# facebookresearch/habitat-lab

Hardware: NVIDIA H100
Metric: DD-PPO learner frames/sec (ResNet18 RGB-D 256x256) (higher is better)
Workload: dtype bf16

## Files before the change

### habitat-lab_b200/csrc/conv.cu

```cuda
#include "common.cuh"
#include "wgmma.cuh"

namespace hb200 {
void count_launch(int n);
static int g_umma_layout = 1;

using namespace wg;

constexpr int kStages = 3;
constexpr int kTileM = 128;
constexpr int kMaxBN = 128;
constexpr int kChunkK = 64;
constexpr int kMaxChunks = 512;

template <int LAYOUT>
__device__ __forceinline__ uint32_t tile_off(int row, int k8, int rows_total) {
  if (LAYOUT == 0) return (uint32_t)(k8 * rows_total + row) << 4;
  return (uint32_t)((row >> 3) << 10) + (uint32_t)((row & 7) << 7) + (uint32_t)((k8 ^ (row & 7)) << 4);
}
template <int LAYOUT>
__device__ __forceinline__ uint64_t kmajor_desc(uint32_t base, int kk, int rows_total) {
  if (LAYOUT == 0)
    return make_smem_desc(base + (uint32_t)(kk * 2 * rows_total * 16), (uint32_t)rows_total * 16, 128, kNoSwizzle);
  return make_smem_desc(base + (uint32_t)(kk * 32), 16, 1024, kSwizzle128B);
}
template <int LAYOUT>
constexpr uint32_t kmajor_hi() { return LAYOUT == 0 ? 8 * 128 : 8 * 1024; }

struct ConvArgs {
  const __nv_bfloat16* src;
  const __nv_bfloat16* wimg;
  __nv_bfloat16* out;
  const __nv_bfloat16* addend;
  double* stats;
  int B, SH, SW, SC;
  int OH, OW, OC;
  int kh, kw, stride, pad;
  int M, nchunks, cshift, gn_groups;
  const float* bias;
  int relu;
  int s2_classes;
  int wbn;
};

template <int BN, int MODE, int LAYOUT, int NST = kStages>
__global__ void __launch_bounds__(128) conv_igemm_kernel(const ConvArgs a) {
  extern __shared__ __align__(16) uint8_t smem_raw[];
  constexpr uint32_t kABytes = kTileM * kChunkK * 2;
  constexpr uint32_t kBBytes = BN * kChunkK * 2;
  constexpr uint32_t kStageBytes = kABytes + kBBytes;
  static_assert(BN <= kMaxBN, "conv: N tile");
  static_assert(NST * kStageBytes >= kStageFloats * sizeof(float), "conv: epilogue transpose buffer");
  const uint32_t smem_base = (smem_u32(smem_raw) + 1023u) & ~1023u;
  float* const stage_buf = reinterpret_cast<float*>(smem_raw + (smem_base - smem_u32(smem_raw)));

  const int tid = threadIdx.x, lane = tid & 31;
  const int n0 = blockIdx.y * BN;
  __shared__ short chunk_ids[kMaxChunks];
  __shared__ int n_valid_s;
  int m, ob, op, oq, ph = 0, pw = 0;
  bool row_ok;
  if (MODE == 1 && a.s2_classes) {
    const int mq = a.M >> 2;
    const int tiles_per_class = (mq + kTileM - 1) / kTileM;
    const int cls = blockIdx.x / tiles_per_class;
    const int idx = (blockIdx.x - cls * tiles_per_class) * kTileM + tid;
    ph = cls >> 1; pw = cls & 1;
    row_ok = idx < mq;
    const int h2 = a.OH >> 1, w2 = a.OW >> 1;
    const int ii = row_ok ? idx : 0;
    ob = ii / (h2 * w2);
    const int rem = ii - ob * (h2 * w2);
    op = 2 * (rem / w2) + ph;
    oq = 2 * (rem % w2) + pw;
    m = (ob * a.OH + op) * a.OW + oq;
  } else {
    m = blockIdx.x * kTileM + tid;
    row_ok = m < a.M;
    const int hw = a.OH * a.OW;
    const int mm = row_ok ? m : 0;
    ob = mm / hw;
    const int rem = mm - ob * hw;
// ... 90 lines not shown
      if (MODE == 0) {
        ih = op * a.stride - a.pad + r;
        iw = oq * a.stride - a.pad + s;
        ok = ok && ih >= 0 && ih < a.SH && iw >= 0 && iw < a.SW;
      } else {
        const int th = op + a.pad - r, tw = oq + a.pad - s;
        ih = th / a.stride;
        iw = tw / a.stride;
        ok = ok && th >= 0 && tw >= 0 && (ih * a.stride == th) && (iw * a.stride == tw) &&
             ih < a.SH && iw < a.SW;
      }
      const __nv_bfloat16* g =
          ok ? a.src + ((((size_t)ob * a.SH + ih) * a.SW + iw) << a.cshift) + c0 : a.src;
      cp_async16(sa + tile_off<LAYOUT>(tid, j, kTileM), g, ok);
    }
    }
    const uint4* wsrc = reinterpret_cast<const uint4*>(wtile + (size_t)chunk * ((size_t)wbn * kChunkK));
#pragma unroll
    for (int i = 0; i < BN / 16; ++i) {
      const int v = tid + i * 128;
      cp_async16(sb + ((uint32_t)v << 4), wsrc + v, true);
    }
  };

  constexpr int kT = MODE == 0 ? kF16 : kBF16;
  float acc_t[BN];
#pragma unroll
  for (int c = 0; c < NST - 1; ++c) {
    if (c < n_valid) load_chunk(chunk_ids[c], c);
    cp_async_commit();
  }
  for (int c = 0; c < n_valid; ++c) {
    const int stage = c % NST;
    cp_async_wait<NST - 2>();
    fence_proxy_async_smem();
    __syncthreads();
    {
      const uint32_t sa = smem_base + stage * kStageBytes;
      const uint32_t sb = sa + kABytes;
      wgmma_fence();
#pragma unroll
      for (int kk = 0; kk < kChunkK / 16; ++kk)
        mma128<BN, kT>(acc_t, kmajor_desc<LAYOUT>(sa, kk, kTileM), kmajor_hi<LAYOUT>(), kmajor_desc<LAYOUT>(sb, kk, BN),
                       (c > 0 || kk > 0) ? 1u : 0u);
      wgmma_commit();
    }
    const int nc = c + NST - 1;
    if (nc < n_valid) {
      wgmma_wait<1>();
      load_chunk(chunk_ids[nc], nc % NST);
    }
    cp_async_commit();
  }
  wgmma_wait<0>();
  acc_fence(acc_t);

  const int hw = a.OH * a.OW;
  int seg = 1;
  if ((hw & (hw - 1)) == 0) seg = hw < 32 ? hw : 32;
#pragma unroll
  for (int col0 = 0; col0 < BN; col0 += 32) {
    float acc[32];
    if (n_valid > 0) {
      acc_row32(acc_t, col0, stage_buf, acc);
    } else {
#pragma unroll
      for (int j = 0; j < 32; ++j) acc[j] = 0.f;
    }

    if (MODE == 0 && a.stats != nullptr) {
      const int cpg = a.OC / a.gn_groups;
      float s2[16], q2[16];
#pragma unroll
      for (int i = 0; i < 16; ++i) {
        s2[i] = acc[2 * i] + acc[2 * i + 1];
        q2[i] = acc[2 * i] * acc[2 * i] + acc[2 * i + 1] * acc[2 * i + 1];
      }
      int lg = 0;
      while ((2 << lg) < cpg && lg < 4) ++lg;
#pragma unroll
      for (int lvl = 0; lvl < 4; ++lvl) {
        if (lvl < lg) {
#pragma unroll
          for (int i = 0; i < (8 >> lvl); ++i) {
            s2[i] = s2[2 * i] + s2[2 * i + 1];
            q2[i] = q2[2 * i] + q2[2 * i + 1];
          }
        }
      }
      const int ng = 16 >> lg;
#pragma unroll
      for (int off = 1; off < 32; off <<= 1) {
        if (off < seg) {
#pragma unroll
          for (int i = 0; i < 16; ++i) {
            if (i < ng) {
              s2[i] += __shfl_xor_sync(0xffffffffu, s2[i], off);
              q2[i] += __shfl_xor_sync(0xffffffffu, q2[i], off);
            }
          }
        }
      }
      if (row_ok && (lane & (seg - 1)) == 0) {
        const int g0 = (n0 + col0) / cpg;
        double* dst = a.stats + ((size_t)ob * a.gn_groups + g0) * 2;
#pragma unroll
        for (int i = 0; i < 16; ++i) {
          if (i < ng) {
            atomicAdd(dst + 2 * i, (double)s2[i]);
            atomicAdd(dst + 2 * i + 1, (double)q2[i]);
          }
        }
      }
    }
    if (MODE == 0 && a.bias != nullptr) {
#pragma unroll
      for (int j = 0; j < 32; ++j) acc[j] += __ldg(a.bias + n0 + col0 + j);
    }
    if (MODE == 0 && a.relu) {
#pragma unroll
      for (int j = 0; j < 32; ++j) acc[j] = fmaxf(acc[j], 0.f);
    }
    if (row_ok) {
      const size_t o = (size_t)m * a.OC + n0 + col0;
      if (MODE == 1 && a.addend != nullptr) {
        const uint4* ad = reinterpret_cast<const uint4*>(a.addend + o);
#pragma unroll
        for (int v = 0; v < 4; ++v) {
          float f[8];
          unpack8(ad[v], f);
#pragma unroll
          for (int e = 0; e < 8; ++e) acc[v * 8 + e] += f[e];
        }
      }
      uint4* dst = reinterpret_cast<uint4*>(a.out + o);
#pragma unroll
      for (int v = 0; v < 4; ++v) {
        uint4 u;
        if (MODE == 0) {
          u.x = pack_f16x2(acc[v * 8 + 0], acc[v * 8 + 1]);
          u.y = pack_f16x2(acc[v * 8 + 2], acc[v * 8 + 3]);
          u.z = pack_f16x2(acc[v * 8 + 4], acc[v * 8 + 5]);
          u.w = pack_f16x2(acc[v * 8 + 6], acc[v * 8 + 7]);
        } else {
          u.x = pack_bf16x2(acc[v * 8 + 0], acc[v * 8 + 1]);
          u.y = pack_bf16x2(acc[v * 8 + 2], acc[v * 8 + 3]);
          u.z = pack_bf16x2(acc[v * 8 + 4], acc[v * 8 + 5]);
          u.w = pack_bf16x2(acc[v * 8 + 6], acc[v * 8 + 7]);
        }
        dst[v] = u;
      }
    }
  }
}

struct WgradArgs {
  const __nv_bfloat16* x;
  const __nv_bfloat16* dy;
  float* dw;
  int B, Hi, Wi, Ci, Ho, Wo, Co, kh, kw, stride, pad;
  int P;
  int KW;
  int chunks_per_split;
  int cshift;
};

template <int BN>
__global__ void __launch_bounds__(128) conv_wgrad_kernel(const WgradArgs a) {
  extern __shared__ __align__(16) uint8_t smem_raw[];
  __shared__ float stage_buf[kStageFloats];
  constexpr uint32_t kABytes = kTileM * kChunkK * 2;
  constexpr uint32_t kBBytes = BN * kChunkK * 2;
  constexpr uint32_t kStageBytes = kABytes + kBBytes;
  constexpr uint32_t kLboA = (kTileM / 8) * 128, kLboB = (BN / 8) * 128;
  static_assert(BN <= kMaxBN, "conv_wgrad: N tile");
  const uint32_t smem_base = (smem_u32(smem_raw) + 1023u) & ~1023u;

  const int tid = threadIdx.x;
  const int row_base = blockIdx.x * kTileM;
  const int n0 = blockIdx.y * BN;
  const long long total_chunks = ((long long)a.P + kChunkK - 1) / kChunkK;
  const long long c_begin = (long long)blockIdx.z * a.chunks_per_split;
  long long c_end = c_begin + a.chunks_per_split;
  if (c_end > total_chunks) c_end = total_chunks;
  const int nchunks = (int)(c_end - c_begin);
  if (nchunks <= 0) return;

  const int kpix = tid & 63;
  const int half = tid >> 6;
  const int taps = a.kh * a.kw;
  const int hw = a.Ho * a.Wo;

  auto load_chunk = [&](int chunk, int stage) {
    const uint32_t sa = smem_base + stage * kStageBytes;
    const uint32_t sb = sa + kABytes;
    const long long pg = (c_begin + chunk) * kChunkK + kpix;
    const bool pix_ok = pg < a.P;
    int b = 0, oh = 0, ow = 0;
    if (pix_ok) {
      b = (int)(pg / hw);
      const int rem = (int)(pg - (long long)b * hw);
      oh = rem / a.Wo;
      ow = rem - oh * a.Wo;
    }
    const uint32_t koff = (uint32_t)(kpix >> 3) * 0 + (uint32_t)((kpix & 7) << 4);
#pragma unroll
    for (int i = 0; i < 8; ++i) {
      const int mb = half * 8 + i;
      const int row0 = row_base + mb * 8;
      const int tap = row0 >> a.cshift;
      const int c0 = row0 & (a.Ci - 1);
      const int r = tap / a.kw, s = tap - r * a.kw;
      const int ih = oh * a.stride - a.pad + r, iw = ow * a.stride - a.pad + s;
      const bool ok = pix_ok && tap < taps && ih >= 0 && ih < a.Hi && iw >= 0 && iw < a.Wi;
      const __nv_bfloat16* g = ok ? a.x + ((((size_t)b * a.Hi + ih) * a.Wi + iw) << a.cshift) + c0 : a.x;
      cp_async16(sa + (uint32_t)(kpix >> 3) * kLboA + (uint32_t)mb * 128 + koff, g, ok);
    }
#pragma unroll
    for (int i = 0; i < BN / 16; ++i) {
      const int nb = half + 2 * i;
      const __nv_bfloat16* g = pix_ok ? a.dy + (size_t)pg * a.Co + n0 + nb * 8 : a.dy;
      cp_async16(sb + (uint32_t)(kpix >> 3) * kLboB + (uint32_t)nb * 128 + koff, g, pix_ok);
    }
  };

  float acc_t[BN];
#pragma unroll
  for (int c = 0; c < kStages - 1; ++c) {
    if (c < nchunks) load_chunk(c, c);
    cp_async_commit();
  }
  for (int c = 0; c < nchunks; ++c) {
    const int stage = c % kStages;
    cp_async_wait<kStages - 2>();
// ... 104 lines not shown
    for (int col0 = 0; col0 < N; col0 += 32) {
      float r[32];
      acc_row32(acc_t, col0, stage_buf, r);
      for (int j = 0; j < 32; ++j) D[(size_t)(m0 + tid) * N + col0 + j] = r[j];
    }
  } else {
    const int w = tid >> 5, l = tid & 31;
#pragma unroll
    for (int h = 0; h < 2; ++h)
#pragma unroll
      for (int i = 0; i < N / 8; ++i) {
        const int row = m0 + h * 64 + 16 * w + (l >> 2), col = 8 * i + 2 * (l & 3);
        const float* f = &acc_t[h * (N / 2) + 4 * i];
        D[(size_t)row * N + col] = f[0];
        D[(size_t)row * N + col + 1] = f[1];
        D[(size_t)(row + 8) * N + col] = f[2];
        D[(size_t)(row + 8) * N + col + 1] = f[3];
      }
  }
}

__global__ void pack_weight_kernel(const float* __restrict__ w, __nv_bfloat16* __restrict__ img,
                                   int rows , int BN, int kc ,
                                   int kc_real, int taps, int kw, int nchunks, int transposed,
                                   int co, int ci_real, int layout) {
  const long long nvec = (long long)(rows / BN) * nchunks * BN * 8;
  for (long long v = blockIdx.x * (long long)blockDim.x + threadIdx.x; v < nvec;
       v += (long long)gridDim.x * blockDim.x) {
    const int per_tile = BN * 8;
    const long long t = v / per_tile;
    const int within = (int)(v - t * per_tile);
    const int ntile = (int)(t / nchunks), chunk = (int)(t - (long long)ntile * nchunks);
    int row, k8;
    if (layout == 0) {
      k8 = within / BN;
      row = within - k8 * BN;
    } else {
      const int g = within >> 6, rr = (within >> 3) & 7, pos = within & 7;
      row = g * 8 + rr;
      k8 = pos ^ rr;
    }
    const int n = ntile * BN + row;
    float f[8];
#pragma unroll
    for (int e = 0; e < 8; ++e) {
      const int k = chunk * kChunkK + k8 * 8 + e;
      const int tap = k / kc, c = k - tap * kc;
      float val = 0.f;
      if (tap < taps && c < kc_real) {
        const int r = tap / kw, s = tap - r * kw;
        const int kh = taps / kw;
        const int o = transposed ? c : n, i = transposed ? n : c;
        if (o < co && i < ci_real) val = w[(((size_t)o * ci_real + i) * kh + r) * kw + s];
      }
      f[e] = val;
    }
    reinterpret_cast<uint4*>(img)[v] = transposed ? pack8(f) : pack8a(f);
  }
}

__global__ void unpack_wgrad_kernel(const float* __restrict__ acc, float* __restrict__ dw, int co,
                                    int ci_real, int ci_pad, int kh, int kw) {
  const long long n = (long long)co * ci_real * kh * kw;
  for (long long i = blockIdx.x * (long long)blockDim.x + threadIdx.x; i < n;
       i += (long long)gridDim.x * blockDim.x) {
    const int s = (int)(i % kw);
    long long t = i / kw;
    const int r = (int)(t % kh);
    t /= kh;
    const int ci = (int)(t % ci_real);
    const int o = (int)(t / ci_real);
    dw[i] = acc[((size_t)(r * kw + s) * ci_pad + ci) * co + o];
  }
}

static int ilog2(int v) {
  int l = 0;
  while ((1 << l) < v) ++l;
  return l;
}
static bool is_pow2(int v) { return v > 0 && (v & (v - 1)) == 0; }
static int pick_bn(int n) { return n >= kMaxBN ? kMaxBN : n; }

template <int MODE>
static int launch_igemm(ConvArgs a, int BN, cudaStream_t st) {
  a.wbn = BN;
  bool deep = false;
  if (g_umma_layout == 1) {
    const int mt = a.s2_classes ? 4 * cdiv(a.M / 4, kTileM) : cdiv(a.M, kTileM);
    while (BN > 32 && 2LL * mt * (a.OC / BN) <= kNumSMs) BN /= 2;
    deep = (long long)mt * (a.OC / BN) <= kNumSMs && a.nchunks > kStages;
  }
  HB_CHECK_ARG(a.nchunks <= kMaxChunks, "conv: K = kh*kw*C = %d exceeds %d", a.nchunks * kChunkK, kMaxChunks * kChunkK);
  dim3 grid(a.s2_classes ? 4 * cdiv(a.M / 4, kTileM) : cdiv(a.M, kTileM), a.OC / BN);
#define HB_CONV_CASE(bn, L, nst)                                                                \
  {                                                                                             \
    const size_t smem = (size_t)(nst) * (kTileM * kChunkK * 2 + bn * kChunkK * 2) + 1024;       \
    auto kern = conv_igemm_kernel<bn, MODE, L, nst>;                                            \
    HB_CUDA(cudaFuncSetAttribute(kern, cudaFuncAttributeMaxDynamicSharedMemorySize, (int)smem)); \
    kern<<<grid, 128, smem, st>>>(a);                                                           \
  }
#define HB_CONV_BN(bn, nst_deep)                                \
  if (g_umma_layout == 0) HB_CONV_CASE(bn, 0, kStages)          \
  else if (deep) HB_CONV_CASE(bn, 1, nst_deep)                  \
  else HB_CONV_CASE(bn, 1, kStages)
  switch (BN) {
    case 32: HB_CONV_BN(32, 8); break;
    case 64: HB_CONV_BN(64, 8); break;
    case 128: HB_CONV_BN(128, 6); break;
    default:
      set_last_error("conv: unsupported N tile %d", BN);
      return HB200_ERR_UNSUPPORTED;
  }
#undef HB_CONV_BN
#undef HB_CONV_CASE
  HB_LAUNCH_OK();
  count_launch(1);
  return HB200_OK;
}

static int check_shape(const hb200_conv_shape* s) {
  HB_CHECK_ARG(s, "conv: null shape");
  HB_CHECK_ARG(s->batch > 0 && s->hi > 0 && s->wi > 0 && s->kh > 0 && s->kw > 0 && s->stride > 0,
               "conv: bad shape");
  HB_CHECK_ARG(is_pow2(s->ci) && s->ci >= 8, "conv: Ci=%d must be a power of two >= 8", s->ci);
  HB_CHECK_ARG(is_pow2(s->co) && s->co >= 32, "conv: Co=%d must be a power of two >= 32", s->co);
  HB_CHECK_ARG(s->ho == (s->hi + 2 * s->pad - s->kh) / s->stride + 1 &&
                   s->wo == (s->wi + 2 * s->pad - s->kw) / s->stride + 1,
               "conv: output dims inconsistent");
  return HB200_OK;
}

}

using namespace hb200;

extern "C" int hb200_set_umma_layout(int layout) {
  HB_CHECK_ARG(layout == 0 || layout == 1, "umma layout must be 0 or 1");
  g_umma_layout = layout;
  return HB200_OK;
}
extern "C" int hb200_get_umma_layout(void) { return g_umma_layout; }

extern "C" int hb200_conv_fwd(const hb200_bf16* x, const hb200_bf16* w_packed, hb200_bf16* y,
                              double* gn_stats, int gn_groups, const hb200_conv_shape* s,
                              hb200_stream_t stream) {
  int rc = check_shape(s);
  if (rc) return rc;
  HB_CHECK_ARG(x && w_packed && y, "conv_fwd: null pointer");
  if (gn_stats) {
    HB_CHECK_ARG(gn_groups > 0 && s->co % gn_groups == 0 && is_pow2(s->co / gn_groups) && s->co / gn_groups >= 2,
                 "conv_fwd: channels per GroupNorm group must be a power of two >= 2");
  }
  ConvArgs a;
  a.src = (const __nv_bfloat16*)x; a.wimg = (const __nv_bfloat16*)w_packed; a.out = (__nv_bfloat16*)y;
  a.addend = nullptr; a.stats = gn_stats;
  a.B = s->batch; a.SH = s->hi; a.SW = s->wi; a.SC = s->ci;
  a.OH = s->ho; a.OW = s->wo; a.OC = s->co;
  a.kh = s->kh; a.kw = s->kw; a.stride = s->stride; a.pad = s->pad;
  a.M = s->batch * s->ho * s->wo;
  a.nchunks = cdiv((long long)s->kh * s->kw * s->ci, kChunkK);
  a.cshift = ilog2(s->ci);
  a.gn_groups = gn_groups > 0 ? gn_groups : 1;
  a.s2_classes = 0;
  a.bias = nullptr;
  a.relu = 0;
  return launch_igemm<0>(a, pick_bn(s->co), (cudaStream_t)stream);
}

// ... 176 lines not shown
```

### habitat-lab_b200/csrc/wgmma.cuh

```cuda
#pragma once
#include <cuda_runtime.h>
#include <stdint.h>

namespace hb200 {
namespace wg {

__device__ __forceinline__ uint32_t smem_u32(const void* p) {
  return (uint32_t)__cvta_generic_to_shared(p);
}

enum Layout : uint32_t { kNoSwizzle = 0, kSwizzle128B = 2, kSwizzle64B = 4 };

__device__ __forceinline__ uint64_t make_smem_desc(uint32_t smem_addr, uint32_t lbo_bytes,
                                                   uint32_t sbo_bytes, uint32_t layout) {
  uint64_t d = 0;
  d |= (uint64_t)((smem_addr >> 4) & 0x3FFF);
  d |= (uint64_t)((lbo_bytes >> 4) & 0x3FFF) << 16;
  d |= (uint64_t)((sbo_bytes >> 4) & 0x3FFF) << 32;
  d |= (uint64_t)(layout & 7) << 61;
  return d;
}
__device__ __forceinline__ uint64_t desc_add(uint64_t d, uint32_t bytes) { return d + (uint64_t)(bytes >> 4); }

constexpr int kF16 = 0, kBF16 = 1, kTF32 = 2;
// ... 104 lines not shown
template <> struct Wgmma<128, kF16 + 0> {
  template <int TA, int TB>
  static __device__ __forceinline__ void mma(float (&d)[64], uint64_t da, uint64_t db, uint32_t accum) {
    asm volatile(
        "{\n\t.reg .pred p;\n\tsetp.ne.b32 p, %66, 0;\n\t"
        "wgmma.mma_async.sync.aligned.m64n128k16.f32.f16.f16 "
        "{%0, %1, %2, %3, %4, %5, %6, %7, %8, %9, %10, %11, %12, %13, %14, %15, %16, %17, %18, %19, %20, %21, %22, %23, %24, %25, %26, %27, %28, %29, %30, %31, %32, %33, %34, %35, %36, %37, %38, %39, %40, %41, %42, %43, %44, %45, %46, %47, %48, %49, %50, %51, %52, %53, %54, %55, %56, %57, %58, %59, %60, %61, %62, %63}, %64, %65, p, 1, 1, %67, %68;\n\t}\n"
        : "+f"(d[0]), "+f"(d[1]), "+f"(d[2]), "+f"(d[3]), "+f"(d[4]), "+f"(d[5]), "+f"(d[6]), "+f"(d[7]), "+f"(d[8]), "+f"(d[9]), "+f"(d[10]), "+f"(d[11]), "+f"(d[12]), "+f"(d[13]), "+f"(d[14]), "+f"(d[15]), "+f"(d[16]), "+f"(d[17]), "+f"(d[18]), "+f"(d[19]), "+f"(d[20]), "+f"(d[21]), "+f"(d[22]), "+f"(d[23]), "+f"(d[24]), "+f"(d[25]), "+f"(d[26]), "+f"(d[27]), "+f"(d[28]), "+f"(d[29]), "+f"(d[30]), "+f"(d[31]), "+f"(d[32]), "+f"(d[33]), "+f"(d[34]), "+f"(d[35]), "+f"(d[36]), "+f"(d[37]), "+f"(d[38]), "+f"(d[39]), "+f"(d[40]), "+f"(d[41]), "+f"(d[42]), "+f"(d[43]), "+f"(d[44]), "+f"(d[45]), "+f"(d[46]), "+f"(d[47]), "+f"(d[48]), "+f"(d[49]), "+f"(d[50]), "+f"(d[51]), "+f"(d[52]), "+f"(d[53]), "+f"(d[54]), "+f"(d[55]), "+f"(d[56]), "+f"(d[57]), "+f"(d[58]), "+f"(d[59]), "+f"(d[60]), "+f"(d[61]), "+f"(d[62]), "+f"(d[63])
        : "l"(da), "l"(db), "r"(accum), "n"(TA), "n"(TB));
  }
};
template <> struct Wgmma<128, kF16 + 1> {
  template <int TA, int TB>
  static __device__ __forceinline__ void mma(float (&d)[64], uint64_t da, uint64_t db, uint32_t accum) {
    asm volatile(
        "{\n\t.reg .pred p;\n\tsetp.ne.b32 p, %66, 0;\n\t"
        "wgmma.mma_async.sync.aligned.m64n128k16.f32.bf16.bf16 "
        "{%0, %1, %2, %3, %4, %5, %6, %7, %8, %9, %10, %11, %12, %13, %14, %15, %16, %17, %18, %19, %20, %21, %22, %23, %24, %25, %26, %27, %28, %29, %30, %31, %32, %33, %34, %35, %36, %37, %38, %39, %40, %41, %42, %43, %44, %45, %46, %47, %48, %49, %50, %51, %52, %53, %54, %55, %56, %57, %58, %59, %60, %61, %62, %63}, %64, %65, p, 1, 1, %67, %68;\n\t}\n"
        : "+f"(d[0]), "+f"(d[1]), "+f"(d[2]), "+f"(d[3]), "+f"(d[4]), "+f"(d[5]), "+f"(d[6]), "+f"(d[7]), "+f"(d[8]), "+f"(d[9]), "+f"(d[10]), "+f"(d[11]), "+f"(d[12]), "+f"(d[13]), "+f"(d[14]), "+f"(d[15]), "+f"(d[16]), "+f"(d[17]), "+f"(d[18]), "+f"(d[19]), "+f"(d[20]), "+f"(d[21]), "+f"(d[22]), "+f"(d[23]), "+f"(d[24]), "+f"(d[25]), "+f"(d[26]), "+f"(d[27]), "+f"(d[28]), "+f"(d[29]), "+f"(d[30]), "+f"(d[31]), "+f"(d[32]), "+f"(d[33]), "+f"(d[34]), "+f"(d[35]), "+f"(d[36]), "+f"(d[37]), "+f"(d[38]), "+f"(d[39]), "+f"(d[40]), "+f"(d[41]), "+f"(d[42]), "+f"(d[43]), "+f"(d[44]), "+f"(d[45]), "+f"(d[46]), "+f"(d[47]), "+f"(d[48]), "+f"(d[49]), "+f"(d[50]), "+f"(d[51]), "+f"(d[52]), "+f"(d[53]), "+f"(d[54]), "+f"(d[55]), "+f"(d[56]), "+f"(d[57]), "+f"(d[58]), "+f"(d[59]), "+f"(d[60]), "+f"(d[61]), "+f"(d[62]), "+f"(d[63])
        : "l"(da), "l"(db), "r"(accum), "n"(TA), "n"(TB));
  }
};
template <> struct Wgmma<128, kTF32> {
  template <int TA, int TB>
  static __device__ __forceinline__ void mma(float (&d)[64], uint64_t da, uint64_t db, uint32_t accum) {
    static_assert(TA == 0 && TB == 0, "tf32 operands are K-major only");
    asm volatile(
        "{\n\t.reg .pred p;\n\tsetp.ne.b32 p, %66, 0;\n\t"
        "wgmma.mma_async.sync.aligned.m64n128k8.f32.tf32.tf32 "
        "{%0, %1, %2, %3, %4, %5, %6, %7, %8, %9, %10, %11, %12, %13, %14, %15, %16, %17, %18, %19, %20, %21, %22, %23, %24, %25, %26, %27, %28, %29, %30, %31, %32, %33, %34, %35, %36, %37, %38, %39, %40, %41, %42, %43, %44, %45, %46, %47, %48, %49, %50, %51, %52, %53, %54, %55, %56, %57, %58, %59, %60, %61, %62, %63}, %64, %65, p, 1, 1;\n\t}\n"
        : "+f"(d[0]), "+f"(d[1]), "+f"(d[2]), "+f"(d[3]), "+f"(d[4]), "+f"(d[5]), "+f"(d[6]), "+f"(d[7]), "+f"(d[8]), "+f"(d[9]), "+f"(d[10]), "+f"(d[11]), "+f"(d[12]), "+f"(d[13]), "+f"(d[14]), "+f"(d[15]), "+f"(d[16]), "+f"(d[17]), "+f"(d[18]), "+f"(d[19]), "+f"(d[20]), "+f"(d[21]), "+f"(d[22]), "+f"(d[23]), "+f"(d[24]), "+f"(d[25]), "+f"(d[26]), "+f"(d[27]), "+f"(d[28]), "+f"(d[29]), "+f"(d[30]), "+f"(d[31]), "+f"(d[32]), "+f"(d[33]), "+f"(d[34]), "+f"(d[35]), "+f"(d[36]), "+f"(d[37]), "+f"(d[38]), "+f"(d[39]), "+f"(d[40]), "+f"(d[41]), "+f"(d[42]), "+f"(d[43]), "+f"(d[44]), "+f"(d[45]), "+f"(d[46]), "+f"(d[47]), "+f"(d[48]), "+f"(d[49]), "+f"(d[50]), "+f"(d[51]), "+f"(d[52]), "+f"(d[53]), "+f"(d[54]), "+f"(d[55]), "+f"(d[56]), "+f"(d[57]), "+f"(d[58]), "+f"(d[59]), "+f"(d[60]), "+f"(d[61]), "+f"(d[62]), "+f"(d[63])
        : "l"(da), "l"(db), "r"(accum));
  }
};

__device__ __forceinline__ void wgmma_fence() { asm volatile("wgmma.fence.sync.aligned;" ::: "memory"); }
__device__ __forceinline__ void wgmma_commit() { asm volatile("wgmma.commit_group.sync.aligned;" ::: "memory"); }
template <int N>
__device__ __forceinline__ void wgmma_wait() {
  asm volatile("wgmma.wait_group.sync.aligned %0;" ::"n"(N) : "memory");
}
template <int N>
__device__ __forceinline__ void acc_fence(float (&acc)[N]) {
#pragma unroll
  for (int i = 0; i < N; ++i) asm volatile("" : "+f"(acc[i])::"memory");
}

template <int N, int T, int TA = 0, int TB = 0>
__device__ __forceinline__ void mma128(float (&acc)[N], uint64_t da, uint32_t a_hi, uint64_t db, uint32_t accum) {
  static_assert(N == 16 || N == 32 || N == 64 || N == 128, "wgmma tile width");
  Wgmma<N, T>::template mma<TA, TB>(*reinterpret_cast<float(*)[N / 2]>(&acc[0]), da, db, accum);
  Wgmma<N, T>::template mma<TA, TB>(*reinterpret_cast<float(*)[N / 2]>(&acc[N / 2]), desc_add(da, a_hi), db, accum);
}

__device__ __forceinline__ void wg_bar_sync(int id) { asm volatile("bar.sync %0, 128;" ::"r"(id) : "memory"); }

constexpr int kStagePitch = 33;
constexpr int kStageFloats = 128 * kStagePitch;
template <int N>
__device__ __forceinline__ void acc_row32(const float (&acc)[N], int col0, float* stage, float (&r)[32], int bar = 1) {
  const int t = threadIdx.x & 127, w = t >> 5, l = t & 31;
  wg_bar_sync(bar);
#pragma unroll
  for (int h = 0; h < 2; ++h) {
#pragma unroll
    for (int i = 0; i < 4; ++i) {
      const int idx = h * (N / 2) + ((col0 >> 3) + i) * 4;
      const int row = h * 64 + 16 * w + (l >> 2), col = 8 * i + 2 * (l & 3);
      stage[row * kStagePitch + col] = acc[idx];
      stage[row * kStagePitch + col + 1] = acc[idx + 1];
      stage[(row + 8) * kStagePitch + col] = acc[idx + 2];
      stage[(row + 8) * kStagePitch + col + 1] = acc[idx + 3];
    }
  }
  wg_bar_sync(bar);
#pragma unroll
  for (int j = 0; j < 32; ++j) r[j] = stage[t * kStagePitch + j];
}

__device__ __forceinline__ void fence_proxy_async_smem() {
  asm volatile("fence.proxy.async.shared::cta;" ::: "memory");
}

__device__ __forceinline__ void mbar_init(uint64_t* bar, uint32_t count) {
  asm volatile("mbarrier.init.shared::cta.b64 [%0], %1;" ::"r"(smem_u32(bar)), "r"(count) : "memory");
}
__device__ __forceinline__ void mbar_fence_init() {
  asm volatile("fence.mbarrier_init.release.cluster;" ::: "memory");
}
__device__ __forceinline__ void mbar_arrive(uint64_t* bar) {
  asm volatile("mbarrier.arrive.shared::cta.b64 _, [%0];" ::"r"(smem_u32(bar)) : "memory");
}
__device__ __forceinline__ bool mbar_try_wait(uint64_t* bar, uint32_t parity) {
  uint32_t ok;
  asm volatile(
      "{\n\t"
      ".reg .pred p;\n\t"
      "mbarrier.try_wait.parity.shared::cta.b64 p, [%1], %2;\n\t"
      "selp.u32 %0, 1, 0, p;\n\t"
      "}\n"
      : "=r"(ok)
      : "r"(smem_u32(bar)), "r"(parity)
      : "memory");
  return ok != 0;
}
__device__ __forceinline__ void mbar_wait(uint64_t* bar, uint32_t parity) {
  if (mbar_try_wait(bar, parity)) return;
  const long long t0 = clock64();
  while (!mbar_try_wait(bar, parity)) {
    if (clock64() - t0 > 4000000000ll) __trap();
  }
}

__device__ __forceinline__ void mbar_expect_tx(uint64_t* bar, uint32_t bytes) {
  asm volatile("mbarrier.arrive.expect_tx.shared::cta.b64 _, [%0], %1;" ::"r"(smem_u32(bar)), "r"(bytes) : "memory");
}
__device__ __forceinline__ void tma_load_4d(uint32_t smem_dst, const void* tmap, uint64_t* bar, int c0, int c1,
                                            int c2, int c3) {
  asm volatile(
      "cp.async.bulk.tensor.4d.shared::cluster.global.tile.mbarrier::complete_tx::bytes [%0], [%1, {%3, %4, %5, %6}], [%2];"
      ::"r"(smem_dst), "l"(reinterpret_cast<uint64_t>(tmap)), "r"(smem_u32(bar)), "r"(c0), "r"(c1), "r"(c2), "r"(c3)
      : "memory");
}

__device__ __forceinline__ void tma_load_5d(uint32_t smem_dst, const void* tmap, uint64_t* bar, int c0, int c1, int c2,
                                            int c3, int c4) {
  asm volatile(
      "cp.async.bulk.tensor.5d.shared::cluster.global.tile.mbarrier::complete_tx::bytes [%0], [%1, {%3, %4, %5, %6, %7}], [%2];"
      ::"r"(smem_dst), "l"(reinterpret_cast<uint64_t>(tmap)), "r"(smem_u32(bar)), "r"(c0), "r"(c1), "r"(c2), "r"(c3),
        "r"(c4)
      : "memory");
}
__device__ __forceinline__ void bulk_load_1d(uint32_t smem_dst, const void* gsrc, uint32_t bytes, uint64_t* bar) {
  asm volatile("cp.async.bulk.shared::cluster.global.mbarrier::complete_tx::bytes [%0], [%1], %2, [%3];" ::"r"(smem_dst),
               "l"(gsrc), "r"(bytes), "r"(smem_u32(bar))
               : "memory");
}
__device__ __forceinline__ void tma_load_2d(uint32_t smem_dst, const void* tmap, uint64_t* bar, int c0, int c1) {
  asm volatile(
      "cp.async.bulk.tensor.2d.shared::cluster.global.tile.mbarrier::complete_tx::bytes [%0], [%1, {%3, %4}], [%2];"
      ::"r"(smem_dst), "l"(reinterpret_cast<uint64_t>(tmap)), "r"(smem_u32(bar)), "r"(c0), "r"(c1)
      : "memory");
}

__device__ __forceinline__ void cp_async16(uint32_t smem_dst, const void* gsrc, bool valid) {
  const uint32_t sz = valid ? 16u : 0u;
  asm volatile("cp.async.cg.shared.global [%0], [%1], 16, %2;" ::"r"(smem_dst), "l"(gsrc), "r"(sz)
               : "memory");
}
__device__ __forceinline__ void cp_async_commit() { asm volatile("cp.async.commit_group;" ::: "memory"); }
template <int N>
__device__ __forceinline__ void cp_async_wait() {
  asm volatile("cp.async.wait_group %0;" ::"n"(N) : "memory");
}

}
}
```

Baseline: 55750.

## Add warp-specialized persistent conv igemm kernel with im2col TMA loads

Adds a persistent, warp-specialized implicit-GEMM conv kernel for stride-1 convs with large output. One producer warpgroup issues im2col TMA loads for activations and bulk loads for weights into a 4-stage mbarrier ring, while two consumer warpgroups run 128x128 wgmma tiles with more registers via setmaxnreg. The aim is to overlap memory transfer with tensor-core math and to remove the software im2col address generation. It depends on the driver im2col tensor-map entry point and adds a new code path with its own register budget, tail handling and statistics epilogue, which could change correctness or occupancy.

```diff
diff --git a/habitat-lab_b200/csrc/conv.cu b/habitat-lab_b200/csrc/conv.cu
--- a/habitat-lab_b200/csrc/conv.cu
+++ b/habitat-lab_b200/csrc/conv.cu
@@ -1,3 +1,5 @@
+#include <cuda.h>
+
 #include "common.cuh"
 #include "wgmma.cuh"
 
@@ -254,9 +256,11 @@
       for (int lvl = 0; lvl < 4; ++lvl) {
         if (lvl < lg) {
 #pragma unroll
-          for (int i = 0; i < (8 >> lvl); ++i) {
-            s2[i] = s2[2 * i] + s2[2 * i + 1];
-            q2[i] = q2[2 * i] + q2[2 * i + 1];
+          for (int i = 0; i < 8; ++i) {
+            if (i < (8 >> lvl)) {
+              s2[i] = s2[2 * i] + s2[2 * i + 1];
+              q2[i] = q2[2 * i] + q2[2 * i + 1];
+            }
           }
         }
       }
@@ -322,6 +326,194 @@
         }
         dst[v] = u;
       }
+    }
+  }
+}
+
+constexpr int kWsThreads = 384;
+constexpr int kWsStages = 4;
+constexpr int kWsProducerRegs = 40;
+constexpr int kWsConsumerRegs = 232;
+
+template <int MODE, bool SPLIT_N>
+__global__ void __launch_bounds__(kWsThreads, 1)
+conv_igemm_kernel(const ConvArgs a, const __grid_constant__ CUtensorMap tmap, int lo_w, int lo_h) {
+  constexpr int BN = kMaxBN;
+  extern __shared__ __align__(16) uint8_t smem_raw[];
+  auto epilogue = [&](const float (&acc_t)[BN], int m, int ob, bool row_ok, int n0, float* stage_buf, int bar) {
+    const int lane = threadIdx.x & 31;
+    const int hw = a.OH * a.OW;
+    int seg = 1;
+    if ((hw & (hw - 1)) == 0) seg = hw < 32 ? hw : 32;
+#pragma unroll
+    for (int col0 = 0; col0 < BN; col0 += 32) {
+      float acc[32];
+      acc_row32(acc_t, col0, stage_buf, acc, bar);
+
+      if (MODE == 0 && a.stats != nullptr) {
+        const int cpg = a.OC / a.gn_groups;
+        float s2[16], q2[16];
+#pragma unroll
+        for (int i = 0; i < 16; ++i) {
+          s2[i] = acc[2 * i] + acc[2 * i + 1];
+          q2[i] = acc[2 * i] * acc[2 * i] + acc[2 * i + 1] * acc[2 * i + 1];
+        }
+        int lg = 0;
+        while ((2 << lg) < cpg && lg < 4) ++lg;
+#pragma unroll
+        for (int lvl = 0; lvl < 4; ++lvl) {
+          if (lvl < lg) {
+#pragma unroll
+            for (int i = 0; i < 8; ++i) {
+              if (i < (8 >> lvl)) {
+                s2[i] = s2[2 * i] + s2[2 * i + 1];
+                q2[i] = q2[2 * i] + q2[2 * i + 1];
+              }
+            }
+          }
+        }
+        const int ng = 16 >> lg;
+#pragma unroll
+        for (int off = 1; off < 32; off <<= 1) {
+          if (off < seg) {
+#pragma unroll
+            for (int i = 0; i < 16; ++i) {
+              if (i < ng) {
+                s2[i] += __shfl_xor_sync(0xffffffffu, s2[i], off);
+                q2[i] += __shfl_xor_sync(0xffffffffu, q2[i], off);
+              }
+            }
+          }
+        }
+        if (row_ok && (lane & (seg - 1)) == 0) {
+          const int g0 = (n0 + col0) / cpg;
+          double* dst = a.stats + ((size_t)ob * a.gn_groups + g0) * 2;
+#pragma unroll
+          for (int i = 0; i < 16; ++i) {
+            if (i < ng) {
+              atomicAdd(dst + 2 * i, (double)s2[i]);
+              atomicAdd(dst + 2 * i + 1, (double)q2[i]);
+            }
+          }
+        }
+      }
+      if (row_ok) {
+        const size_t o = (size_t)m * a.OC + n0 + col0;
+        if (MODE == 1 && a.addend != nullptr) {
+          const uint4* ad = reinterpret_cast<const uint4*>(a.addend + o);
+#pragma unroll
+          for (int v = 0; v < 4; ++v) {
+            float f[8];
+            unpack8(ad[v], f);
+#pragma unroll
+            for (int e = 0; e < 8; ++e) acc[v * 8 + e] += f[e];
+          }
+        }
+        uint4* dst = reinterpret_cast<uint4*>(a.out + o);
+#pragma unroll
+        for (int v = 0; v < 4; ++v) {
+          uint4 u;
+          if (MODE == 0) {
+            u.x = pack_f16x2(acc[v * 8 + 0], acc[v * 8 + 1]);
+            u.y = pack_f16x2(acc[v * 8 + 2], acc[v * 8 + 3]);
+            u.z = pack_f16x2(acc[v * 8 + 4], acc[v * 8 + 5]);
+            u.w = pack_f16x2(acc[v * 8 + 6], acc[v * 8 + 7]);
+          } else {
+            u.x = pack_bf16x2(acc[v * 8 + 0], acc[v * 8 + 1]);
+            u.y = pack_bf16x2(acc[v * 8 + 2], acc[v * 8 + 3]);
+            u.z = pack_bf16x2(acc[v * 8 + 4], acc[v * 8 + 5]);
+            u.w = pack_bf16x2(acc[v * 8 + 6], acc[v * 8 + 7]);
+          }
+          dst[v] = u;
+        }
+      }
+    }
+  };
+  constexpr int MT = SPLIT_N ? 1 : 2, NT = SPLIT_N ? 2 : 1;
+  constexpr uint32_t kSub = kTileM * kChunkK * 2;
+  constexpr uint32_t kABytes = MT * kSub, kStageBytes = (MT + NT) * kSub;
+  __shared__ __align__(8) uint64_t full_bar[kWsStages], empty_bar[kWsStages];
+  const uint32_t sbase = (smem_u32(smem_raw) + 1023u) & ~1023u;
+  float* const stage_bufs =
+      reinterpret_cast<float*>(smem_raw + (sbase + kWsStages * kStageBytes - smem_u32(smem_raw)));
+  const int tid = threadIdx.x, wg_id = tid >> 7;
+  if (tid == 0) {
+#pragma unroll
+    for (int i = 0; i < kWsStages; ++i) {
+      mbar_init(&full_bar[i], 1);
+      mbar_init(&empty_bar[i], 2);
+    }
+    mbar_fence_init();
+  }
+  __syncthreads();
+  const int mtiles = (a.M + MT * kTileM - 1) / (MT * kTileM), ntiles = a.OC / (NT * kTileM);
+  const int total = mtiles * ntiles;
+  const int first = blockIdx.x, stride = gridDim.x;
+  const int my_n = first < total ? (total - first + stride - 1) / stride : 0;
+  const int hw = a.OH * a.OW;
+
+  if (wg_id == 0) {
+    setmaxnreg_dec<kWsProducerRegs>();
+    if (tid == 0) {
+      const CUtensorMap* const tmap_p = &tmap;
+      int it = 0;
+      for (int i = 0; i < my_n; ++i) {
+        const int tile = first + i * stride;
+        const int mt = tile / ntiles, nt = tile - mt * ntiles;
+        const int m0 = mt * MT * kTileM;
+        const int ob = m0 / hw, rem = m0 - ob * hw;
+        const int oh = rem / a.OW, ow = rem - oh * a.OW;
+        const int w0 = ow * a.stride + lo_w, h0 = oh * a.stride + lo_h;
+        const __nv_bfloat16* wsrc = a.wimg + (size_t)nt * NT * a.nchunks * (kTileM * kChunkK);
+        for (int c = 0; c < a.nchunks; ++c, ++it) {
+          const int st = it % kWsStages;
+          if (it >= kWsStages) mbar_wait(&empty_bar[st], ((it / kWsStages) - 1) & 1);
+          const int k0 = c * kChunkK;
+          const int tap = k0 >> a.cshift, c0 = k0 & (a.SC - 1);
+          const int r = tap / a.kw, s = tap - r * a.kw;
+          const int offw = MODE == 0 ? s : a.kw - 1 - s, offh = MODE == 0 ? r : a.kh - 1 - r;
+          const uint32_t sa = sbase + (uint32_t)st * kStageBytes;
+          mbar_expect_tx(&full_bar[st], kStageBytes);
+          tma_load_im2col_4d(sa, tmap_p, &full_bar[st], c0, w0, h0, ob, (uint16_t)offw, (uint16_t)offh);
+#pragma unroll
+          for (int j = 0; j < NT; ++j)
+            bulk_load_1d(sa + kABytes + j * kSub, wsrc + ((size_t)j * a.nchunks + c) * (kTileM * kChunkK), kSub,
+                         &full_bar[st]);
+        }
+      }
+    }
+  } else {
+    setmaxnreg_inc<kWsConsumerRegs>();
+    constexpr int kT = MODE == 0 ? kF16 : kBF16;
+    const int wgi = wg_id - 1, t = tid & 127;
+    const uint32_t a_off = SPLIT_N ? 0u : (uint32_t)wgi * kSub;
+    const uint32_t b_off = kABytes + (SPLIT_N ? (uint32_t)wgi * kSub : 0u);
+    float* const stage_buf = stage_bufs + wgi * kStageFloats;
+    float acc_t[kMaxBN];
+    int it = 0;
+    for (int i = 0; i < my_n; ++i) {
+      const int tile = first + i * stride;
+      const int mt = tile / ntiles, nt = tile - mt * ntiles;
+      for (int c = 0; c < a.nchunks; ++c, ++it) {
+        const int st = it % kWsStages;
+        mbar_wait(&full_bar[st], (it / kWsStages) & 1);
+        const uint32_t sa = sbase + (uint32_t)st * kStageBytes;
+        wgmma_fence();
+#pragma unroll
+        for (int kk = 0; kk < kChunkK / 16; ++kk)
+          mma128<kMaxBN, kT>(acc_t, kmajor_desc<1>(sa + a_off, kk, kTileM), kmajor_hi<1>(),
+                             kmajor_desc<1>(sa + b_off, kk, kMaxBN), (c > 0 || kk > 0) ? 1u : 0u);
+        wgmma_commit();
+        wgmma_wait<1>();
+        if (c > 0 && t == 0) mbar_arrive(&empty_bar[(it - 1) % kWsStages]);
+      }
+      wgmma_wait<0>();
+      acc_fence(acc_t);
+      if (t == 0) mbar_arrive(&empty_bar[(it - 1) % kWsStages]);
+      const int m = mt * MT * kTileM + (SPLIT_N ? 0 : wgi * kTileM) + t;
+      const bool row_ok = m < a.M;
+      const int n0 = (nt * NT + (SPLIT_N ? wgi : 0)) * kTileM;
+      epilogue(acc_t, m, (row_ok ? m : 0) / hw, row_ok, n0, stage_buf, 1 + wgi);
     }
   }
 }
@@ -592,9 +784,81 @@
 static bool is_pow2(int v) { return v > 0 && (v & (v - 1)) == 0; }
 static int pick_bn(int n) { return n >= kMaxBN ? kMaxBN : n; }
 
+typedef CUresult (*EncodeIm2colFn)(CUtensorMap*, CUtensorMapDataType, cuuint32_t, void*, const cuuint64_t*,
+                                   const cuuint64_t*, const int*, const int*, cuuint32_t, cuuint32_t, const cuuint32_t*,
+                                   CUtensorMapInterleave, CUtensorMapSwizzle, CUtensorMapL2promotion,
+                                   CUtensorMapFloatOOBfill);
+static EncodeIm2colFn im2col_encode_fn() {
+  static EncodeIm2colFn fn = nullptr;
+  if (fn) return fn;
+  void* p = nullptr;
+  cudaDriverEntryPointQueryResult q;
+  if (cudaGetDriverEntryPoint("cuTensorMapEncodeIm2col", &p, cudaEnableDefault, &q) != cudaSuccess ||
+      q != cudaDriverEntryPointSuccess)
+    return nullptr;
+  fn = (EncodeIm2colFn)p;
+  return fn;
+}
+
+static void im2col_corners(int src_dim, int n, int step, int lo, int* lower, int* upper) {
+  *lower = lo;
+  *upper = lo + (n - 1) * step - (src_dim - 1);
+}
+
+template <int MODE, bool SPLIT_N>
+static int launch_igemm_ws(const ConvArgs& a, cudaStream_t st) {
+  constexpr int MT = SPLIT_N ? 1 : 2;
+  EncodeIm2colFn enc = im2col_encode_fn();
+  if (!enc) {
+    set_last_error("conv (im2col TMA): cuTensorMapEncodeIm2col is not available from this driver");
+    return HB200_ERR_UNSUPPORTED;
+  }
+  const int step = MODE == 0 ? a.stride : 1;
+  const int lo_h = MODE == 0 ? -a.pad : -(a.kh - 1 - a.pad), lo_w = MODE == 0 ? -a.pad : -(a.kw - 1 - a.pad);
+  int lower[2], upper[2];
+  im2col_corners(a.SW, a.OW, step, lo_w, &lower[0], &upper[0]);
+  im2col_corners(a.SH, a.OH, step, lo_h, &lower[1], &upper[1]);
+  CUtensorMap tmap;
+  const cuuint64_t dims[4] = {(cuuint64_t)a.SC, (cuuint64_t)a.SW, (cuuint64_t)a.SH, (cuuint64_t)a.B};
+  const cuuint64_t strides[3] = {(cuuint64_t)a.SC * 2, (cuuint64_t)a.SW * a.SC * 2, (cuuint64_t)a.SH * a.SW * a.SC * 2};
+  const cuuint32_t estr[4] = {1u, (cuuint32_t)step, (cuuint32_t)step, 1u};
+  const CUresult r = enc(&tmap, CU_TENSOR_MAP_DATA_TYPE_BFLOAT16, 4, (void*)a.src, dims, strides, lower, upper,
+                         (cuuint32_t)kChunkK, (cuuint32_t)(MT * kTileM), estr, CU_TENSOR_MAP_INTERLEAVE_NONE,
+                         CU_TENSOR_MAP_SWIZZLE_128B, CU_TENSOR_MAP_L2_PROMOTION_L2_128B, CU_TENSOR_MAP_FLOAT_OOB_FILL_NONE);
+  if (r != CUDA_SUCCESS) {
+    set_last_error("conv (im2col TMA): cuTensorMapEncodeIm2col failed (%d)", (int)r);
+    return HB200_ERR_CUDA;
+  }
+  const size_t smem = (size_t)kWsStages * 3 * kTileM * kChunkK * 2 + 2 * kStageFloats * sizeof(float) + 1024;
+  auto kern = conv_igemm_kernel<MODE, SPLIT_N>;
+  static int grid_cache = 0;
+  if (grid_cache == 0) {
+    HB_CUDA(cudaFuncSetAttribute(kern, cudaFuncAttributeMaxDynamicSharedMemorySize, (int)smem));
+    cudaFuncAttributes fa;
+    HB_CUDA(cudaFuncGetAttributes(&fa, (const void*)kern));
+    const int regs = fa.numRegs > 0 ? fa.numRegs : 168;
+    int per_sm = 65536 / (((regs + 7) / 8 * 8) * kWsThreads);
+    const int by_smem = (int)((227 * 1024) / (smem + fa.sharedSizeBytes));
+    if (by_smem < per_sm) per_sm = by_smem;
+    if (per_sm < 1) per_sm = 1;
+    grid_cache = kNumSMs * per_sm;
+  }
+  const int tiles = cdiv(a.M, MT * kTileM) * (a.OC / ((SPLIT_N ? 2 : 1) * kTileM));
+  const int grid = grid_cache < tiles ? grid_cache : tiles;
+  kern<<<grid, kWsThreads, smem, st>>>(a, tmap, lo_w, lo_h);
+  HB_LAUNCH_OK();
+  count_launch(1);
+  return HB200_OK;
+}
+
 template <int MODE>
 static int launch_igemm(ConvArgs a, int BN, cudaStream_t st) {
   a.wbn = BN;
+  if (g_umma_layout == 1 && BN == kMaxBN && a.SC % kChunkK == 0 && !a.s2_classes && a.stride == 1 &&
+      a.bias == nullptr && !a.relu && 2LL * cdiv(a.M, kTileM) * (a.OC / kMaxBN) > kNumSMs) {
+    if (a.OC >= 2 * kMaxBN) return launch_igemm_ws<MODE, true>(a, st);
+    return launch_igemm_ws<MODE, false>(a, st);
+  }
   bool deep = false;
   if (g_umma_layout == 1) {
     const int mt = a.s2_classes ? 4 * cdiv(a.M / 4, kTileM) : cdiv(a.M, kTileM);
diff --git a/habitat-lab_b200/csrc/wgmma.cuh b/habitat-lab_b200/csrc/wgmma.cuh
--- a/habitat-lab_b200/csrc/wgmma.cuh
+++ b/habitat-lab_b200/csrc/wgmma.cuh
@@ -210,6 +210,15 @@
   asm volatile("fence.proxy.async.shared::cta;" ::: "memory");
 }
 
+template <int R>
+__device__ __forceinline__ void setmaxnreg_dec() {
+  asm volatile("setmaxnreg.dec.sync.aligned.u32 %0;" ::"n"(R));
+}
+template <int R>
+__device__ __forceinline__ void setmaxnreg_inc() {
+  asm volatile("setmaxnreg.inc.sync.aligned.u32 %0;" ::"n"(R));
+}
+
 __device__ __forceinline__ void mbar_init(uint64_t* bar, uint32_t count) {
   asm volatile("mbarrier.init.shared::cta.b64 [%0], %1;" ::"r"(smem_u32(bar)), "r"(count) : "memory");
 }
@@ -259,6 +268,15 @@
         "r"(c4)
       : "memory");
 }
+__device__ __forceinline__ void tma_load_im2col_4d(uint32_t smem_dst, const void* tmap, uint64_t* bar, int c, int w,
+                                                   int h, int n, uint16_t off_w, uint16_t off_h) {
+  asm volatile(
+      "cp.async.bulk.tensor.4d.shared::cluster.global.im2col.mbarrier::complete_tx::bytes [%0], [%1, {%3, %4, %5, %6}], "
+      "[%2], {%7, %8};"
+      ::"r"(smem_dst), "l"(reinterpret_cast<uint64_t>(tmap)), "r"(smem_u32(bar)), "r"(c), "r"(w), "r"(h), "r"(n),
+        "h"(off_w), "h"(off_h)
+      : "memory");
+}
 __device__ __forceinline__ void bulk_load_1d(uint32_t smem_dst, const void* gsrc, uint32_t bytes, uint64_t* bar) {
   asm volatile("cp.async.bulk.shared::cluster.global.mbarrier::complete_tx::bytes [%0], [%1], %2, [%3];" ::"r"(smem_dst),
                "l"(gsrc), "r"(bytes), "r"(smem_u32(bar))
```

Measured after the change: 58340, median of 6. 4.7% higher.
